# tuneinsight/lattigo

Hardware: AMD Instinct MI355X
Metric: ciphertext-mul+relin ops/s (higher is better)
Workload: dtype u64; 1 GPU; BGV logN=15, 12 Q-limbs [55,45x11] + 3 P-limbs [55x3], T=65537: ct x ct MulRelin (tensor + gadget product + ModDown), inputs resident in HBM; batch_per_gpu=256, logN=15, L=12, alpha=3, beta=4, parallelism=1 independent replicas, ciphertext-sharded

## Files before the change

### lattigo_amd/csrc/api.cpp

```cpp
#include <hip/hip_runtime.h>

#include <algorithm>
#include <atomic>
#include <chrono>
#include <condition_variable>
#include <deque>
#include <functional>
#include <cstdarg>
#include <cstdio>
#include <cstring>
#include <map>
#include <memory>
#include <tuple>
#include <mutex>
#include <shared_mutex>
#include <string>
#include <thread>
#include <unordered_map>
#include <unordered_set>
#include <cstdlib>
#include <vector>
#include <dlfcn.h>
#include <pthread.h>
#include <sched.h>
// ... 3025 lines not shown
    return mx != 0 && modup_f64_raw_ok(be.Q->logN, nsrc, mx);
}
struct MacDigits {
    const uint64_t *dec = nullptr;
    size_t bs = 0, ds = 0;
    bool raw = false, own_reduce = true;
};
struct TensorIn {
    View a0, a1, b0, b1;
    const uint64_t *ts;
};
struct LazyArgs {
    View cx;
    int B = 0;
    View c0Q, c0P, c1Q, c1P;
    bool cx_canonical = false;
    const TensorIn *tin = nullptr;
    const KsScatter *giant = nullptr;
    MacDigits *pending = nullptr;
};
int ks_mac_f64(Evaluator &ev, int levelQ, const Evk &k, const KsRoute &r, const LazyArgs &m, const MacDigits &dec, const NttMacEpilogue *epi) {
    BasisExtender &be = *ev.be;
    const hipStream_t st = be.ctx->stream;
    const int levelP = k.nPk - 1, N = be.Q->N;
    NttMacArgs a{};
    a.beta = base_rns_size(levelQ, levelP);
    key_product_limbs(a, be, k, levelQ, levelP, 2);
    a.dec_dstride = dec.ds;
    a.key_kstride = (size_t)(k.nQk + k.nPk) * N;
    a.key_dstride = 2 * a.key_kstride;
    a.own_alpha = levelP + 1;
    a.own_nq = levelQ + 1;
    a.own_reduce = dec.own_reduce ? 1 : 0;
    a.dec_f64 = dec.raw ? 1 : 0;
    a.q_out_f64 = 0;
    const View decv{const_cast<uint64_t *>(dec.dec), dec.bs};
    if (epi) {
        NttMacEpilogue e = *epi;
        for (int i = 0; i < a.nlimbs; i++) { e.sp[i] = epi->sp[a.out_limb[i]]; e.tsp[i] = epi->tsp[a.out_limb[i]]; }
        HIP_TRY(launch_ntt_mac_f64(be.qp, a, decv, m.cx, k.keyd, m.c0Q, m.c0P, m.c1Q, m.c1P, m.B, st, &e));
        return HE_OK;
    }
    if (!r.acc_q_f64) {
        HIP_TRY(launch_ntt_mac_f64(be.qp, a, decv, m.cx, k.keyd, m.c0Q, m.c0P, m.c1Q, m.c1P, m.B, st, nullptr, m.giant));
        return HE_OK;
    }
    NttMacArgs aq = a, ap = a;
    key_product_limbs(aq, be, k, levelQ, -1, 2);
    key_product_limbs(ap, be, k, -1, levelP, 2);
    aq.q_out_f64 = 1;
    HIP_TRY(launch_ntt_mac_f64(be.qp, aq, decv, m.cx, k.keyd, m.c0Q, m.c0P, m.c1Q, m.c1P, m.B, st));
    HIP_TRY(launch_ntt_mac_f64(be.qp, ap, decv, m.cx, k.keyd, m.c0Q, m.c0P, m.c1Q, m.c1P, m.B, st));
    return HE_OK;
}
struct KsCall {
    KsRoute route;
    const FusedPlan *dec = nullptr, *md = nullptr;
};
int rgsw_nj(const Evk &k, int i) { return k.pw2 ? k.nj[i] : 1; }
int window_products_core(Evaluator &ev, int levelQ, const Evk &k, const LazyArgs &a, bool reduce_wide) {
    BasisExtender &be = *ev.be;
    const int levelP = k.nPk - 1, N = be.Q->N, B = a.B;
    int beta = 0;
    for (int i = 0; i <= levelQ; i++) beta += rgsw_nj(k, i);
    const size_t wq = (size_t)B * (levelQ + 1) * N, ds = (size_t)(be.LQ + be.LP) * N, bs = (size_t)beta * ds;
    View inv{be.ctx->arena_take(wq), (size_t)(levelQ + 1) * N};
// ... 24 lines not shown
    return ks_inner(ev, levelQ, levelP, View{dec, bs}, ds, k, a.c0Q, a.c0P, a.c1Q, a.c1P, B);
}
int gadget_product_lazy_core(Evaluator &ev, int levelQ, const Evk &k, const KsCall &c, const LazyArgs &a) {
    BasisExtender &be = *ev.be;
    const KsRoute &r = c.route;
    const int levelP = k.nPk - 1, N = be.Q->N, B = a.B;
    const int beta = key_beta(k, levelQ);
    const size_t wq = (size_t)B * (levelQ + 1) * N, ds = (size_t)(be.LQ + be.LP) * N, bs = (size_t)beta * ds;
    const View cx = a.cx;
    if (a.tin) {
        LimbTab tt;
        QPLimb l[kMaxLimbs];
        uint64_t tsv[kMaxLimbs];
        tt.n = qp_limbs(be, levelQ, -1, r.prod_prologue ? 1 : 0, l);
        for (int i = 0; i < tt.n; i++) {
            tt.in_limb[i] = tt.out_limb[i] = tt.mod[i] = l[i].mod;
            tsv[i] = a.tin->ts[l[i].mod];
        }
        if (tt.n > 0)
            HIP_TRY(launch_tensor(be.qp, tt, tsv, a.tin->a0, a.tin->a1, a.tin->b0, a.tin->b1, View{nullptr, 0}, View{nullptr, 0}, cx, B, be.ctx->stream));
    }
    if (r.digits == KS_DIGITS_WINDOWS) return window_products_core(ev, levelQ, k, a, false);
    uint64_t *cxinv = be.ctx->arena_take(wq);
    uint64_t *dec = be.ctx->arena_take((size_t)B * bs);
    View inv{cxinv, (size_t)(levelQ + 1) * N};
    if (r.digits == KS_DIGITS_UNFUSED) {
        HIP_TRY(be_ntt(be, ident_tab(levelQ + 1), cx, inv, B, true, NTT_REDUCE_INPUT));
        TRY(decompose_ntt_into(ev, levelQ, levelP, levelP + 1, cx, inv, View{dec, bs}, ds, B));
        return ks_inner(ev, levelQ, levelP, View{dec, bs}, ds, k, a.c0Q, a.c0P, a.c1Q, a.c1P, B);
    }
    if (r.prod_prologue) {
        NttProdIn pin;
        pin.a = a.tin->a1; pin.b = a.tin->b1; pin.c = cx;
        for (int i = 0; i <= levelQ; i++) pin.ts[i] = a.tin->ts[i];
        HIP_TRY(launch_ntt_rows(be.qp, ident_tab(levelQ + 1), cx, inv, B, true, 0, be.ctx->stream, nullptr, &pin));
    } else {
        HIP_TRY(launch_ntt_rows(be.qp, ident_tab(levelQ + 1), cx, inv, B, true, a.cx_canonical ? 0 : NTT_REDUCE_INPUT, be.ctx->stream));
    }
    if (!r.mac_f64) {
        TRY(decompose_fused(ev, *c.dec, levelQ, levelP, levelP + 1, inv, View{dec, bs}, B));
        return ks_inner(ev, levelQ, levelP, View{dec, bs}, ds, k, a.c0Q, a.c0P, a.c1Q, a.c1P, B, &cx, levelP + 1, 0, 0, -1, a.giant);
    }
    int max_nsrc = 1;
    for (const FusedGroup &g : c.dec->groups) max_nsrc = std::max(max_nsrc, g.nsrc);
    const MacDigits digits{dec, bs, ds, f64_raw_ok(be, levelQ, levelP, max_nsrc), !a.cx_canonical};
    TRY(decompose_fused(ev, *c.dec, levelQ, levelP, levelP + 1, inv, View{dec, bs}, B, 1, digits.raw));
    TRY(ks_inner(ev, levelQ, levelP, View{dec, bs}, ds, k, a.c0Q, a.c0P, a.c1Q, a.c1P, B, &cx, levelP + 1, 1, 0, -1, a.giant));
    if (r.moddown == KS_MD_FUSED_MAC) {
        *a.pending = digits;
        return HE_OK;
    }
    return ks_mac_f64(ev, levelQ, k, r, a, digits, nullptr);
}
int moddown_front_fused(Evaluator &ev, const FusedPlan &plan, int levelQ, int levelP, View accP, View sP, View sQ, int nb, bool canonical, bool *raw) {
    BasisExtender &be = *ev.be;
    hipStream_t st = be.ctx->stream;
    HIP_TRY(launch_ntt_rows(be.qp, ident_tab(levelP + 1, 0, 0, be.LQ), accP, sP, nb, true, canonical ? 0 : NTT_REDUCE_INPUT, st));
    const FusedGroup &g = plan.groups[0];
    *raw = f64_raw_ok(be, levelQ, -1, g.nsrc);
    HIP_TRY(launch_modup_fused(be.qp, g.dev, 1, g.nsrc, g.dst_classes, sP, sQ, sQ, nb, st, *raw, g.total_limbs));
    return HE_OK;
}
void moddown_epilogue(NttEpilogue &epi, const BasisExtender &be, int levelP, const LimbTab &tab, View y) {
    for (int i = 0; i < tab.n; i++) epi.s[i] = be.Q->moduli[tab.mod[i]] - be.md_ptoq[levelP][tab.mod[i]];
    epi.y = y; epi.has_w = false; epi.w = y;
}
// ... 69 lines not shown
    epi.has_w = g.add0 != nullptr; epi.w = g.add0 ? *g.add0 : a0Q;
    epi.y_small_f64 = r.acc_q_f64;
    epi.zsplit = B; epi.out2 = g.out1; epi.y2 = a1Q; epi.has_w2 = g.add1 != nullptr; epi.w2 = g.add1 ? *g.add1 : a1Q;
    if (g.tin) {
        epi.tensor = true; epi.has_w = epi.has_w2 = false;
        epi.ta0 = g.tin->a0; epi.ta1 = g.tin->a1; epi.tb0 = g.tin->b0; epi.tb1 = g.tin->b1;
        for (int i = 0; i < ti.n; i++) epi.ts[i] = g.tin->ts[ti.mod[i]];
    }
    if (mac_epilogue) {
        NttMacEpilogue me;
        me.scatter_ginv = g.scatter_ginv;
        me.ext = sQ; me.ext_f64 = raw;
        me.out0 = g.out0; me.out1 = g.out1;
        me.has_w0 = g.add0 != nullptr && !g.tin; me.has_w1 = g.add1 != nullptr && !g.tin;
        me.w0 = g.add0 ? *g.add0 : g.out0; me.w1 = g.add1 ? *g.add1 : g.out1;
        me.tensor = g.tin != nullptr;
        if (g.tin) { me.ta0 = g.tin->a0; me.ta1 = g.tin->a1; me.tb0 = g.tin->b0; me.tb1 = g.tin->b1; }
        for (int i = 0; i <= levelQ; i++) {
            const ModConst &m = be.Q->sub[i].mc;
            me.sp[i] = (double)imform(be.Q->moduli[i] - be.md_ptoq[levelP][i], m.q, m.qinv);
            me.tsp[i] = g.tin ? (double)imform(imform(g.tin->ts[i], m.q, m.qinv), m.q, m.qinv) : 0.0;
        }
        TRY(ks_mac_f64(ev, levelQ, k, r, lazy, pending, &me));
    }
    if (ti.n > 0) HIP_TRY(launch_ntt_rows(be.qp, ti, sQ, g.out0, 2 * B, false, (raw && !mac_epilogue) ? NTT_INPUT_F64 : 0, st, &epi));
    return HE_OK;
}
int ks_call(Evaluator &ev, KsForm form, int levelQ, const Evk &k, KsAlias alias, KsCall *out) {
    static const bool no_mac_epilogue = env_flag("HERING_NO_MAC_EPILOGUE");
    static const bool no_prod_prologue = env_flag("HERING_NO_PROD_PROLOGUE");
    static const bool no_tensor_epilogue = env_flag("HERING_NO_TENSOR_EPILOGUE");
    static const bool no_auto_scatter = env_flag("HERING_NO_AUTO_SCATTER");
    static const bool no_giant_fusion = env_flag("HERING_NO_GIANT_FUSION");
    const BasisExtender &be = *ev.be;
    const int logN = be.Q->logN;
    KsFacts f;
    f.form = form; f.ring_type = be.type; f.levelP = k.nPk - 1;
    f.pw2 = k.pw2 != 0; f.keyd = k.keyd != nullptr; f.f64_tables = be.d_twdi != nullptr;
    for (int j = 0; j < k.nPk; j++) f.p_class2 = f.p_class2 || be.small[be.LQ + j] == 2;
    const bool lazy = form == KS_LAZY || form == KS_GIANT_STEP || form == KS_AUTOMORPHISM_HOISTED_LAZY;
    if (k.nPk > 0 && !k.pw2 && form != KS_HOISTED && form != KS_AUTOMORPHISM_HOISTED_LAZY) TRY(get_dec_plan(ev, levelQ, k.nPk - 1, k.nPk, &out->dec));
    if (k.nPk > 0 && !lazy) TRY(get_md_plan(ev, levelQ, k.nPk - 1, &out->md));
    f.dec_ok = out->dec && out->dec->ok; f.md_ok = out->md && out->md->ok;
    f.prod_in_supported = ntt_prod_in_supported(logN); f.scatter_supported = epilogue_scatter_supported(logN);
    f.mac_epilogue_supported = ntt_mac_epilogue_supported(logN); f.mac_giant_supported = ntt_mac_giant_supported(logN);
    f.alias = alias;
    f.no_mac_epilogue = no_mac_epilogue; f.no_prod_prologue = no_prod_prologue; f.no_tensor_epilogue = no_tensor_epilogue;
    f.no_auto_scatter = no_auto_scatter; f.no_giant_fusion = no_giant_fusion;
    out->route = ks_route(f);
    return HE_OK;
}
int key_switch(Evaluator &ev, KsForm form, int levelQ, const Evk &k, KsAlias alias, const GpArgs &g) {
    KsCall c;
    TRY(ks_call(ev, form, levelQ, k, alias, &c));
    return gadget_product_core(ev, levelQ, k, c, g);
}
void ks_request(CoReq &q, int op, std::shared_ptr<Evaluator> ev, std::shared_ptr<Evk> k, int level, KsForm form, KsAlias alias) {
    q.op = op; q.obj = ev.get(); q.key = k.get(); q.par[0] = level;
    q.keep.push_back(ev); q.keep.push_back(k);
    if (!k || form == KS_FORM_COUNT) return;
    q.tables_ok = [ev, k, form, level, alias](bool *ok) -> int {
        KsCall c;
        TRY(ks_call(*ev, form, level, *k, alias, &c));
        *ok = c.route.tables_ok;
        return HE_OK;
    };
}
int check_key(const Evaluator &ev, const Evk &k, int &levelQ, const char *who) {
    if (k.ev.get() != &ev) return fail(HE_EINVAL, "%s: key belongs to another evaluator", who);
    if (levelQ < 0) return fail(HE_EINVAL, "%s: negative level", who);
    levelQ = std::min(levelQ, k.nQk - 1);
    return HE_OK;
}
int check_decomp(const Evaluator &ev, const Decomp &dec, int levelQ, int levelP, const char *who) {
    if (dec.ev.get() != &ev) return fail(HE_EINVAL, "%s: decomposition buffer belongs to another evaluator", who);
    if (dec.fillQ < 0) return fail(HE_EINVAL, "%s: decomposition buffer was never filled", who);
    if (levelP != dec.fillP || levelQ > dec.fillQ || base_rns_size(levelQ, levelP) > dec.fill_beta)
        return fail(HE_EINVAL, "%s: decomposition buffer holds %d digits of level (%d,%d), (%d,%d) requested", who, dec.fill_beta,
                    dec.fillQ, dec.fillP, levelQ, levelP);
    return HE_OK;
}
// ... 2146 lines not shown
```

### lattigo_amd/csrc/kernels.h

```cpp
#pragma once

#include <hip/hip_runtime.h>
#include <stdint.h>
#include <cstdlib>

#include "modarith.h"

namespace he {

inline bool env_flag(const char *name) {
    const char *v = std::getenv(name);
    return v != nullptr && std::atoi(v) != 0;
}
constexpr int kMaxLimbs = 64;
constexpr int kMaxLogN = 20;

struct LimbTab {
    int n;
    uint8_t in_limb[kMaxLimbs];
    uint8_t out_limb[kMaxLimbs];
    uint8_t mod[kMaxLimbs];
};

struct View {
// ... 13 lines not shown
    const double *twd_fwd;
    const double *twd_inv;
    const uint64_t *tws_fwd = nullptr;
};

enum NttFlags {
    NTT_REDUCE_INPUT = 1,
    NTT_LAZY_OUT = 2,
    NTT_ADD_SCALAR = 4,
    NTT_INPUT_F64 = 8,
};
struct NttEpilogue;
hipError_t launch_ntt(const RingDev &r, const LimbTab &tab, View in, View out, int batch, bool inverse, int flags,
                      hipStream_t s, const uint64_t *io_scalar = nullptr, const NttEpilogue *epi = nullptr);
struct NttEpilogue {
    View y, w;
    bool has_w;
    uint64_t s[kMaxLimbs];
    bool y_small_f64 = false;
    bool y_reduce = false;
    int zsplit = 0;
    View out2, y2, w2;
    bool has_w2 = false;
    bool tensor = false;
    View ta0, ta1, tb0, tb1;
    uint64_t ts[kMaxLimbs];
    bool has_dst = false;
    View dst;
    uint32_t scatter_ginv = 0;
};
struct NttProdIn {
    View a, b, c;
    uint64_t ts[kMaxLimbs];
};
int ntt_row_bits(int logN);
bool ntt_prod_in_supported(int logN);
bool epilogue_scatter_supported(int logN);
hipError_t launch_ntt_rows(const RingDev &r, const LimbTab &tab, View in, View out, int batch, bool inverse, int flags,
                           hipStream_t s, const NttEpilogue *epi = nullptr, const NttProdIn *prod = nullptr);

hipError_t launch_ci_fold(const RingDev &r, const LimbTab &tab, View in, View out, int batch, bool inverse, bool reduce_input,
                          hipStream_t s);

hipError_t launch_ci_intt_lazy_ref(const RingDev &r, const ModConst &mc_host, int mod, View in, View out, int batch, hipStream_t s);

enum EwOp {
    EW_ADD = 0, EW_ADD_LAZY, EW_SUB, EW_SUB_LAZY,
    EW_MUL_BARRETT, EW_MUL_BARRETT_LAZY, EW_MUL_BARRETT_THEN_ADD, EW_MUL_BARRETT_THEN_ADD_LAZY,
    EW_MUL_MONT, EW_MUL_MONT_LAZY, EW_MUL_MONT_LAZY_THEN_NEG,
    EW_MUL_MONT_THEN_ADD, EW_MUL_MONT_THEN_ADD_LAZY, EW_MUL_MONT_LAZY_THEN_ADD_LAZY,
    EW_MUL_MONT_THEN_SUB, EW_MUL_MONT_THEN_SUB_LAZY, EW_MUL_MONT_LAZY_THEN_SUB_LAZY,
    EW_NEG = 100, EW_REDUCE, EW_REDUCE_LAZY, EW_MFORM, EW_MFORM_LAZY, EW_IMFORM, EW_COPY,
    EW_ZERO,
    EW_ADD_SCALAR = 200,
    EW_SUB_SCALAR,
    EW_MUL_SCALAR_MONT,
    EW_MUL_SCALAR_MONT_THEN_ADD,
    EW_ADD_SCALAR_LAZY,
    EW_SUB_THEN_MUL_SCALAR_MONT_2Q = 300,
    EW_DIVROUND_COEFF,
    EW_SUBMUL2Q_THEN_ADD,
};
struct ScalarTab {
    uint64_t s[kMaxLimbs];
    uint64_t s2[kMaxLimbs];
};
// ... 100 lines not shown
    int own_nq;
};
struct KsScatter {
    uint32_t ginv = 0;
    View add0{nullptr, 0};
    uint64_t add_s[kMaxLimbs];
    int plain = 0;
    View add0P{nullptr, 0};
    int accumulate = 0;
};
hipError_t launch_ks_inner(const RingDev &r, const KsArgs &a, View dec, View own, const uint64_t *key, View out0Q,
                           View out0P, View out1Q, View out1P, int batch, hipStream_t s, const KsScatter *sc = nullptr);

constexpr int kMaxDiag = 64;
struct DiagMacArgs {
    int n, nlimbs, accumulate;
    int mod0;
    const uint64_t *pt[kMaxDiag], *c0[kMaxDiag], *c1[kMaxDiag];
    const uint32_t *index[kMaxDiag];
    size_t pt_bs[kMaxDiag], c0_bs[kMaxDiag], c1_bs[kMaxDiag];
    const size_t *term_tab = nullptr;
    int term_rows = 3;
};
hipError_t launch_diag_mac(const RingDev &r, const DiagMacArgs &a, View out0, View out1, int batch, hipStream_t s);

struct NttMacArgs {
    int beta, nlimbs;
    uint8_t dec_limb[kMaxLimbs], key_limb[kMaxLimbs], out_limb[kMaxLimbs], out_view[kMaxLimbs], mod[kMaxLimbs];
    size_t dec_dstride, key_kstride, key_dstride;
    int own_alpha, own_nq;
    int dec_f64;
    int own_reduce;
    int q_out_f64;
};
struct NttMacEpilogue {
    View ext;
    bool ext_f64 = false;
    View out0, out1;
    bool has_w0 = false, has_w1 = false;
    View w0, w1;
    bool tensor = false;
    View ta0, ta1, tb0, tb1;
    double sp[kMaxLimbs], tsp[kMaxLimbs];
    uint32_t scatter_ginv = 0;
};
bool ntt_mac_epilogue_supported(int logN);
struct KsScatter;
hipError_t launch_ntt_mac_f64(const RingDev &r, const NttMacArgs &a, View dec, View own, const double *keyd, View out0Q,
                              View out0P, View out1Q, View out1P, int batch, hipStream_t s, const NttMacEpilogue *epi = nullptr,
                              const KsScatter *giant = nullptr);
bool ntt_mac_giant_supported(int logN);
hipError_t launch_key_to_f64(const RingDev &r, const uint64_t *key, double *keyd, int nblocks, const uint8_t *limb_mod_host,
                             int nlimbs, hipStream_t s);

struct RingSwitchIO {
    View in, out;
    View in2{nullptr, 0}, out2{nullptr, 0};
    int zsplit = -1;
};
hipError_t launch_ring_degree_fold_ntt(const RingDev &large, const LimbTab &tab, const uint64_t *gapinv_mont, RingSwitchIO io,
                                       int n_small, int log_gap, int batch, hipStream_t s);
hipError_t launch_ring_degree_replicate_ntt(const LimbTab &tab, RingSwitchIO io, int n_small, int log_gap, int batch, hipStream_t s);
hipError_t launch_ring_degree_stride(const LimbTab &tab, RingSwitchIO io, int n_small, int log_gap, bool up, int batch, hipStream_t s);
hipError_t launch_ci_bridge_fold(const RingDev &moduli, const LimbTab &tab, RingSwitchIO io, int n, int batch, hipStream_t s);
hipError_t launch_ci_bridge_unfold(const LimbTab &tab, RingSwitchIO io, int n, int batch, hipStream_t s);

// ... 32 lines not shown
```

### lattigo_amd/csrc/kernels.hip

```cpp
#include "kernels.h"

#include <atomic>
#include <cstdio>
#include <cstdlib>
#include <type_traits>
#include <mutex>
#include <unordered_map>
#include <vector>

namespace he {

namespace {
struct ProfRec { int id; hipEvent_t e0, e1; double bytes; };
struct ProfState { std::vector<ProfRec> recs; };
std::mutex g_prof_mu;
std::atomic<int> g_prof_active{0};
std::unordered_map<hipStream_t, ProfState> g_prof;
std::vector<hipEvent_t> g_prof_pool;
hipEvent_t prof_event_locked() {
    if (!g_prof_pool.empty()) { hipEvent_t e = g_prof_pool.back(); g_prof_pool.pop_back(); return e; }
    hipEvent_t e;
    (void)hipEventCreate(&e);
    return e;
}
// ... 172 lines not shown

struct NttArgs {
    const uint64_t *in;
    uint64_t *out;
    size_t in_bs, out_bs;
    const ModConst *mc;
    const uint64_t *tw;
    const double *twd;
    int N;
    int a;
    int flags;
    int scale;
    LimbTab tab;
    int epi;
    const uint64_t *epi_y, *epi_w;
    size_t epi_y_bs, epi_w_bs;
    uint64_t epi_s[kMaxLimbs];
    int zsplit;
    int epi2;
    uint64_t *out2;
    size_t out2_bs;
    const uint64_t *epi_y2, *epi_w2;
    size_t epi_y2_bs, epi_w2_bs;
    int epi_tensor;
    const uint64_t *ta0, *ta1, *tb0, *tb1;
    size_t ta0_bs, ta1_bs, tb0_bs, tb1_bs;
    uint64_t epi_ts[kMaxLimbs];
    uint64_t io_s[kMaxLimbs];
    int epi_y_f64;
    int epi_y_reduce;
    int nbatch, iters;
    int nbatch_prof = 0;
    int tprod = 0;
    unsigned sc_ginv = 0;
    int sc_logN = 0;
    const size_t *in_tab = nullptr;
    int cb = 0;
    const size_t *out_tab = nullptr, *out2_tab = nullptr, *epi_w_tab = nullptr, *epi_w2_tab = nullptr;
    const size_t *ta0_tab = nullptr, *ta1_tab = nullptr, *tb0_tab = nullptr, *tb1_tab = nullptr;
    const size_t *epi_y_tab = nullptr, *epi_y2_tab = nullptr;
};

__device__ __forceinline__ int lds_phys(int e) { return e + (e >> 4); }

__device__ __forceinline__ void wave_lds_sync() {
    __builtin_amdgcn_fence(__ATOMIC_RELEASE, "wavefront");
    __builtin_amdgcn_wave_barrier();
    __builtin_amdgcn_fence(__ATOMIC_ACQUIRE, "wavefront");
}
__device__ __forceinline__ void rows_sync(int sh) {
    if (sh <= 6) wave_lds_sync();
    else __syncthreads();
}
template <int T>
__device__ __forceinline__ int nat_e(int k, int tau) {
    constexpr int CH = T >= 64 ? 64 : T;
    return (tau / CH) * (16 * CH) + k * CH + (tau % CH);
}

int ntt_row_bits(int n) {
    return n <= 12 ? n : (n <= 15 ? 12 : 13);
}

template <int G4, bool INV, bool NC>
__device__ __forceinline__ void rows_round(uint64_t (&x)[16], const uint64_t *__restrict__ tw, int rowtw, int s0, int hi0,
                                           int tau, int sh, uint64_t q, uint64_t twoq, uint64_t qinv, const ModConst &mc,
                                           bool scale_last) {
    constexpr int g = G4, G = 1 << g, W = 16 / G;
    if constexpr (!INV) {
#pragma unroll
        for (int u = 0; u < g; u++) {
            const int d = 1 << (g - 1 - u);
#pragma unroll
            for (int w = 0; w < W; w++) {
                const int hi = (W == 1) ? hi0 : ((tau * W + w) >> sh);
                const int base = (rowtw << (s0 + u)) + (hi << u);
// ... 538 lines not shown
#pragma unroll
                for (int k = 0; k < 16; k++) wv[k] = ldnt(&wp[nat_e<T>(k, tau)]);
#pragma unroll
                for (int k = 0; k < 16; k++) {
                    const int e = nat_e<T>(k, tau);
                    const uint64_t v = canon_f64(modmul_f64(lds[lds_phys(e)] - yv[k], sp, q, qi), q, qi);
                    uint64_t *dp = &op[e];
                    if constexpr (SCAT) dp = op - (size_t)row * N2 + auto_dest((unsigned)(row * N2 + e), A.sc_ginv, A.sc_logN);
                    stnt(dp, cred(wv[k] + v, mc.q));
                }
            } else {
#pragma unroll
                for (int k = 0; k < 16; k++) {
                    const int e = nat_e<T>(k, tau);
                    uint64_t *dp = &op[e];
                    if constexpr (SCAT) dp = op - (size_t)row * N2 + auto_dest((unsigned)(row * N2 + e), A.sc_ginv, A.sc_logN);
                    stnt(dp, canon_f64(modmul_f64(lds[lds_phys(e)] - yv[k], sp, q, qi), q, qi));
                }
            }
        } else {
#pragma unroll
            for (int k = 0; k < 16; k++) {
                const int e = nat_e<T>(k, tau);
                dst[e] = canon_f64(lds[lds_phys(e)], q, qi);
            }
        }
    } else {
        if constexpr (TP) {
            const size_t off = (size_t)il * A.N + (size_t)row * N2;
            const uint64_t *pa = A.ta1 + voff(A.ta1_tab, A.ta1_bs, bzi) + off, *pb = A.tb1 + voff(A.tb1_tab, A.tb1_bs, bzi) + off;
            uint64_t *pc = A.out2 + (size_t)bzi * A.out2_bs + off;
            const double tsp = (double)imform(imform(A.epi_ts[y], mc.q, mc.qinv), mc.q, mc.qinv);
            const uint64_t twoq_u = mc.q << 1;
#pragma unroll
            for (int h = 0; h < 2; h++) {
                uint64_t ua[8], ub[8];
#pragma unroll
                for (int k = 0; k < 8; k++) { const int e = nat_e<T>(8 * h + k, tau); ua[k] = ldnt(&pa[e]); ub[k] = ldnt(&pb[e]); }
                bool big = false;
#pragma unroll
                for (int k = 0; k < 8; k++) big = big || ua[k] >= twoq_u || ub[k] >= twoq_u;
                if (__any(big)) {
#pragma unroll
                    for (int k = 0; k < 8; k++) { ua[k] = bred_add_lazy(ua[k], mc.q, mc.brc0); ub[k] = bred_add_lazy(ub[k], mc.q, mc.brc0); }
                }
#pragma unroll
                for (int k = 0; k < 8; k++) {
                    const int e = nat_e<T>(8 * h + k, tau);
                    const double c = canon_f64d(modmul_f64(modmul_f64(u52_to_f64(ua[k]), u52_to_f64(ub[k]), q, qi), tsp, q, qi), q, qi);
                    stnt(&pc[e], f64_to_u52(c));
                    lds[lds_phys(e)] = c;
                }
            }
        } else {
        if (A.flags & NTT_REDUCE_INPUT) {
            const uint64_t twoq_u = mc.q << 1;
            bool big = false;
#pragma unroll
            for (int k = 0; k < 16; k++) big = big || nx[k] >= twoq_u;
            if (__any(big)) {
#pragma unroll
                for (int k = 0; k < 16; k++) nx[k] = bred_add_lazy(nx[k], mc.q, mc.brc0);
            }
        }
#pragma unroll
        for (int k = 0; k < 16; k++) lds[lds_phys(nat_e<T>(k, tau))] = u52_to_f64(nx[k]);
        }
        if constexpr (PIPE) if (bzi + 1 < b1) {
            const uint64_t *srcn = A.in + voff(A.in_tab, A.in_bs, bzi + 1) + in_off;
#pragma unroll
            for (int k = 0; k < 16; k++) nx[k] = ldnt(&srcn[nat_e<T>(k, tau)]);
        }
        rows_sync(0);
        if constexpr (GREM > 0) {
            constexpr int s0 = 4 * NR4;
            rows_lds_xfer_f64<LOGB, GREM>(x, lds, tau, s0, 0, false);
            rows_round_f64<GREM, true>(x, tw, rowtw, s0, 0, tau, 0, q, qi);
            rows_lds_xfer_f64<LOGB, GREM>(x, lds, tau, s0, 0, true);
            rows_sync(GREM);
        }
        double t16[15];
        if constexpr (NR4 > 0) rows_tw16_f64(t16, tw, rowtw, 4 * (NR4 - 1), tau >> (LOGB - 4 * NR4));
#pragma unroll 1
        for (int rho = NR4 - 1; rho >= 0; rho--) {
// ... 265 lines not shown
        return A.m.own_alpha > 0 && !it.isP && it.ql >= d * A.m.own_alpha && it.ql < (d + 1) * A.m.own_alpha;
    };
    const int nd = A.m.beta + (EPI ? 2 : 0);
    auto digit_src = [&](const Item &it, int d) -> const uint64_t * {
        if (EPI && d >= A.m.beta)
            return AA.e.ext + ((size_t)(d - A.m.beta) * AA.nbatch + it.bz) * AA.e.ext_bs + (size_t)it.ql * A.N + it.rowoff;
        return own_digit(it, d) ? A.own + voff(A.own_tab, A.own_bs, it.bz) + (size_t)it.ql * A.N + it.rowoff
                                : A.dec + it.bz * A.dec_bs + (size_t)d * A.m.dec_dstride + (size_t)it.ql * A.N + it.rowoff;
    };
    const unsigned pw_addr = lds_byte_addr(pbuf) + wv * 8192u;
    auto dma_digit = [&](const uint64_t *src, unsigned lane) {
        const uint64_t *gp = src + ((lane >> 5) * T + 64u * wv + 2u * (lane & 31u));
#pragma unroll
        for (int j = 0; j < 8; j++) glds16(gp + (size_t)j * 2 * T, pw_addr + (unsigned)j * 1024u);
    };

    unsigned t = 0;
    unsigned w = item_of(0);
    if (w == ~0u) return;
    Item cur = decode(w);
    dma_digit(digit_src(cur, 0), lane);
    for (;;) {
        const unsigned t_cur = t; (void)t_cur;
        MAC_STAMP2(0);
        double acc0[16], acc1[16];
#pragma unroll
        for (int k = 0; k < 16; k++) { acc0[k] = 0.0; acc1[k] = 0.0; }
        const double q = cur.q, qi = cur.qi;
        if (tau < 240u) {
            const unsigned hi = tau / 15u, idx = tau - hi * 15u, u = 31u - (unsigned)__builtin_clz(idx + 1u), j = idx + 1u - (1u << u);
            tw1s[tau] = cur.tw[((unsigned)cur.rowtw << (4 + u)) + (hi << u) + j];
        }
        bool more = false;
        auto round0 = [&](double (&x)[16]) {
            double t0[15];
#pragma unroll
            for (int u = 0; u < 4; u++)
#pragma unroll
                for (int j = 0; j < (1 << u); j++) t0[(1 << u) - 1 + j] = ldcd(cur.tw, (size_t)(((unsigned)cur.rowtw << u) + j));
            rows_round16_f64<false>(x, t0, q, qi);
        };
        auto round1 = [&](double (&x)[16], unsigned tau) {
            rows_lds_xfer_f64<LOGB, 4>(x, lds, tau, 4, LOGB - 8, false);
            {
                double t1[15];
                const double *tp = tw1s + (tau >> (LOGB - 8)) * 15u;
#pragma unroll
                for (int i = 0; i < 15; i++) t1[i] = tp[i];
                rows_round16_f64<false>(x, t1, q, qi);
            }
            rows_lds_xfer_f64<LOGB, 4>(x, lds, tau, 4, LOGB - 8, true);
            rows_sync(LOGB - 8);
            rows_lds_xfer_f64<LOGB, 4>(x, lds, tau, 8, LOGB - 12, false);
        };
        auto transform = [&](int nk, double (&x)[16], unsigned tau, unsigned lane, const uint64_t *nsrc, const double *k0p,
                             const double *k1p, double (&kk0)[16], double (&kk1)[16]) {
            double t2[15];
            rows_tw16_f64(t2, cur.tw, cur.rowtw, 8, tau >> (LOGB - 12));
            __builtin_amdgcn_sched_barrier(0);
            asm volatile("s_waitcnt lgkmcnt(0)" ::: "memory");
            if (nsrc) dma_digit(nsrc, lane);
            __builtin_amdgcn_sched_barrier(0);
            round0(x);
            __syncthreads();
            rows_lds_xfer_f64<LOGB, 4>(x, lds, tau, 0, LOGB - 4, true);
            __syncthreads();
// ... 23 lines not shown
            w = item_of(++t);
            more = w != ~0u;
            return more ? digit_src(decode(w), 0) : nullptr;
        };
        for (int d = 0; d < A.m.beta; d++) {
            const bool is_own = own_digit(cur, d);
            unsigned tau_d = threadIdx.x;
            asm volatile("" : "+v"(tau_d));
            const unsigned tau = tau_d, lane = tau & 63u;
            const double *pw = pbuf + wv * 1024u + lane;
            MAC_STAMP2(1 + d * 12 + 0);
            asm volatile("s_waitcnt vmcnt(0)" ::: "memory");
            uint64_t xi[16];
#pragma unroll
            for (int k = 0; k < 16; k++) xi[k] = (uint64_t)__double_as_longlong(pw[k * 64]);
            double x[16];
            if (is_own && A.m.own_reduce) {
#pragma unroll
                for (int k = 0; k < 16; k++) xi[k] = bred_add_lazy(xi[k], ldc(reinterpret_cast<const uint64_t *>(A.mc + cur.mi), 0), ldc(reinterpret_cast<const uint64_t *>(A.mc + cur.mi), 2));
            }
            if (A.m.dec_f64 && !is_own) {
#pragma unroll
                for (int k = 0; k < 16; k++) x[k] = __longlong_as_double((long long)xi[k]);
            } else {
#pragma unroll
                for (int k = 0; k < 16; k++) x[k] = u52_to_f64(xi[k]);
            }
            MAC_STAMP2(1 + d * 12 + 1);
            const uint64_t *nsrc = next_src(d);
            const double *k0p = cur.kbase + (size_t)d * A.m.key_dstride + tau, *k1p = k0p + A.m.key_kstride;
            double kk0[16], kk1[16];
            if (!is_own) {
                transform(2, x, tau, lane, nsrc, k0p, k1p, kk0, kk1);
            } else {
                asm volatile("s_waitcnt lgkmcnt(0)" ::: "memory");
                if (nsrc) dma_digit(nsrc, lane);
                __builtin_amdgcn_sched_barrier(0);
#pragma unroll
                for (int k = 0; k < 16; k++) kk0[k] = k0p[(unsigned)(k * T)];
#pragma unroll
                for (int k = 0; k < 16; k++) kk1[k] = k1p[(unsigned)(k * T)];
                __builtin_amdgcn_sched_barrier(0);
                __syncthreads();
                rows_lds_xfer_f64<LOGB, 4>(x, lds, tau, 0, LOGB - 4, true);
                __syncthreads();
                mac_final_xfer<LOGB>(x, lds, tau, false);
            }
            MAC_STAMP2(1 + d * 12 + 8);
#pragma unroll
            for (int k = 0; k < 16; k++) acc0[k] += modmul_f64(x[k], kk0[k], q, qi);
            MAC_STAMP2(1 + d * 12 + 9);
#pragma unroll
            for (int k = 0; k < 16; k++) acc1[k] += modmul_f64(x[k], kk1[k], q, qi);
            MAC_STAMP2(1 + d * 12 + 10);
        }
        if constexpr (EPI && TEN && LOGB == 12) {
            unsigned tau_d = threadIdx.x;
            asm volatile("" : "+v"(tau_d));
            const unsigned tau = tau_d, lane = tau & 63u;
            const double *pw = pbuf + wv * 1024u + lane;
            MAC_STAMP2(48);
            asm volatile("s_waitcnt vmcnt(0)" ::: "memory");
            double xA[16], xB[16];
            uint64_t wB[16];
#pragma unroll
            for (int k = 0; k < 16; k++) xA[k] = pw[k * 64];
            const uint64_t *srcB = digit_src(cur, A.m.beta + 1) + tau;
            const uint64_t *nsrc = next_src(A.m.beta + 1);
#pragma unroll
            for (int k = 0; k < 16; k++) wB[k] = ldnt(&srcB[(unsigned)(k * T)]);
            double t2[15];
            rows_tw16_f64(t2, cur.tw, cur.rowtw, 8, tau);
            __builtin_amdgcn_sched_barrier(0);
            asm volatile("s_waitcnt lgkmcnt(0)" ::: "memory");
            if (nsrc) dma_digit(nsrc, lane);
            __builtin_amdgcn_sched_barrier(0);
            if (!AA.e.ext_f64) {
#pragma unroll
                for (int k = 0; k < 16; k++) xA[k] = u52_to_f64((uint64_t)__double_as_longlong(xA[k]));
// ... 221 lines not shown
                ext_pass(std::integral_constant<int, 1>{});
            } else {
#pragma unroll 1
                for (int c = 0; c < 2; c++) ext_pass(c);
            }
        }
        const int ol = cur.out_limb;
        uint64_t *o0 = nullptr, *o1 = nullptr;
        unsigned tau_t = threadIdx.x;
        asm volatile("" : "+v"(tau_t));
        const unsigned tau = tau_t;
        if constexpr (!EPI) {
            o0 = (cur.isP ? A.o0P + voff(A.oP0_tab, A.oP0_bs, cur.bz) : A.o0Q + voff(A.oQ0_tab, A.oQ0_bs, cur.bz)) + (size_t)ol * A.N + cur.rowoff + tau;
            o1 = (cur.isP ? A.o1P + voff(A.oP1_tab, A.oP1_bs, cur.bz) : A.o1Q + voff(A.oQ1_tab, A.oQ1_bs, cur.bz)) + (size_t)ol * A.N + cur.rowoff + tau;
        }
        [[maybe_unused]] uint64_t gs_av[16], gs_p0[16], gs_p1[16];
        [[maybe_unused]] const uint64_t *gs_ap = nullptr;
        if constexpr (!EPI && SCAT) {
            __builtin_amdgcn_sched_barrier(0);
            const size_t src = cur.rowoff + tau;
            if (AA.e.has_w0) gs_ap = (cur.isP ? AA.e.w1 + meoff(AA.e, ME_W1, AA.e.w1_bs, cur.bz, AA.nbatch) : AA.e.w0 + meoff(AA.e, ME_W0, AA.e.w0_bs, cur.bz, AA.nbatch)) + (size_t)ol * A.N + src;
            if (gs_ap) {
#pragma unroll
                for (int k = 0; k < 16; k++) gs_av[k] = ldnt(&gs_ap[(unsigned)(k * T)]);
            }
            if (AA.e.gs_accum) {
                const uint64_t *b0p = o0 - src;
#pragma unroll
                for (int k = 0; k < 16; k++) gs_p0[k] = b0p[auto_dest((unsigned)src + (unsigned)(k * T), AA.e.sc_ginv, AA.e.sc_logN)];
            }
            __builtin_amdgcn_sched_barrier(0);
        }
        if constexpr (!EPI) {
            auto to_natural = [&](double (&a)[16]) {
                mac_final_xfer<LOGB>(a, lds, tau, true);
                __syncthreads();
#pragma unroll
                for (int k = 0; k < 16; k++) a[k] = lds[lds_phys(k * T + tau)];
            };
            to_natural(acc0);
            if constexpr (SCAT) {
                const uint64_t qu = ldc(reinterpret_cast<const uint64_t *>(A.mc + cur.mi), 0);
                const size_t src = cur.rowoff + tau;
                uint64_t *b0p = o0 - src;
                const uint64_t *b1p = o1 - src;
                const bool accum = AA.e.gs_accum != 0;
                if (accum) {
#pragma unroll
                    for (int k = 0; k < 16; k++) gs_p1[k] = b1p[auto_dest((unsigned)src + (unsigned)(k * T), AA.e.sc_ginv, AA.e.sc_logN)];
                }
                __builtin_amdgcn_sched_barrier(0);
#pragma unroll
                for (int k = 0; k < 16; k++) {
                    uint64_t v0 = canon_f64(acc0[k], q, qi);
                    if (gs_ap) v0 = cred(v0 + gs_av[k], qu);
                    if (accum) v0 += gs_p0[k];
                    stnt(&b0p[auto_dest((unsigned)src + (unsigned)(k * T), AA.e.sc_ginv, AA.e.sc_logN)], v0);
                }
            }
            __syncthreads();
            to_natural(acc1);
        }
        if constexpr (EPI) {
            (void)o0; (void)o1; (void)ol;
        } else if constexpr (SCAT) {
            const size_t src = cur.rowoff + tau;
// ... 30 lines not shown
        int dev = 0, n = 0;
        if (hipGetDevice(&dev) != hipSuccess || hipDeviceGetAttribute(&n, hipDeviceAttributeMultiprocessorCount, dev) != hipSuccess || n <= 0)
            n = 256;
        return (unsigned)n;
    }();
    return logb >= 13 ? cus : 2u * cus;
}

bool ntt_prod_in_supported(int logN) {
    const int b = ntt_row_bits(logN);
    return b == 12 || b == 13;
}
bool epilogue_scatter_supported(int logN) {
    const int b = ntt_row_bits(logN);
    return b == 12 || b == 13;
}
bool ntt_mac_epilogue_supported(int logN) {
    const int b = ntt_row_bits(logN);
    return b == 12 || b == 13;
}
bool ntt_mac_giant_supported(int logN) {
    const int b = ntt_row_bits(logN);
    return b == 12 || b == 13;
}
hipError_t launch_ntt_mac_f64(const RingDev &r, const NttMacArgs &a, View dec, View own, const double *keyd, View out0Q,
                              View out0P, View out1Q, View out1P, int batch, hipStream_t s, const NttMacEpilogue *epi,
                              const KsScatter *giant) {
    if (a.nlimbs <= 0 || batch <= 0) return hipSuccess;
    if (!r.twd_fwd || !keyd) return hipErrorInvalidValue;
    if (giant && (epi || a.q_out_f64 || !giant->ginv || !ntt_mac_giant_supported(r.logN))) return hipErrorInvalidValue;
    if (dec.tab || (epi && epi->ext.tab) || (a.q_out_f64 && !no_tab({out0Q, out1Q}))) return hipErrorInvalidValue;
    const int b = ntt_row_bits(r.logN), aa = r.logN - b;
    if (epi && !ntt_mac_epilogue_supported(r.logN)) return hipErrorInvalidValue;
    NttMacKArgs A{};
    A.dec = dec.p; A.dec_bs = dec.bstride; A.own = own.p; A.own_bs = own.bstride; A.own_tab = own.tab; A.keyd = keyd;
    A.o0Q = out0Q.p; A.o0P = out0P.p; A.o1Q = out1Q.p; A.o1P = out1P.p;
    A.oQ0_bs = out0Q.bstride; A.oP0_bs = out0P.bstride; A.oQ1_bs = out1Q.bstride; A.oP1_bs = out1P.bstride;
    A.oQ0_tab = out0Q.tab; A.oP0_tab = out0P.tab; A.oQ1_tab = out1Q.tab; A.oP1_tab = out1P.tab;
    A.mc = r.mc; A.twd = r.twd_fwd; A.N = r.N; A.a = aa; A.m = a;
    double mac_bytes = ((double)a.beta * batch + 2.0 * a.beta + 2.0 * batch) * a.nlimbs * (double)r.N * 8.0;
    if (epi) mac_bytes += (2.0 + (epi->tensor ? 4.0 : (epi->has_w0 ? 1.0 : 0.0) + (epi->has_w1 ? 1.0 : 0.0))) * batch * a.nlimbs * (double)r.N * 8.0;
    if (epi || giant || b >= 12) {
        NttMacDmaArgs D;
        D.k = A;
        D.e = MacEpiK{};
        if (epi) {
            D.e.ext = epi->ext.p; D.e.ext_bs = epi->ext.bstride; D.e.ext_f64 = epi->ext_f64 ? 1 : 0;
            D.e.out0 = epi->out0.p; D.e.out0_bs = epi->out0.bstride; D.e.out1 = epi->out1.p; D.e.out1_bs = epi->out1.bstride;
            D.e.has_w0 = epi->has_w0 ? 1 : 0; D.e.has_w1 = epi->has_w1 ? 1 : 0;
            D.e.w0 = epi->w0.p; D.e.w0_bs = epi->w0.bstride; D.e.w1 = epi->w1.p; D.e.w1_bs = epi->w1.bstride;
            D.e.tensor = epi->tensor ? 1 : 0;
            if (epi->scatter_ginv && epi->tensor) return hipErrorInvalidValue;
            D.e.sc_ginv = epi->scatter_ginv; D.e.sc_logN = r.logN;
            D.e.ta0 = epi->ta0.p; D.e.ta0_bs = epi->ta0.bstride; D.e.ta1 = epi->ta1.p; D.e.ta1_bs = epi->ta1.bstride;
            D.e.tb0 = epi->tb0.p; D.e.tb0_bs = epi->tb0.bstride; D.e.tb1 = epi->tb1.p; D.e.tb1_bs = epi->tb1.bstride;
            {
                const View *vs[8] = {&epi->out0, &epi->out1, &epi->w0, &epi->w1, &epi->ta0, &epi->ta1, &epi->tb0, &epi->tb1};
                const size_t *base = nullptr;
                for (const View *v : vs) if (v->tab && (!base || v->tab < base)) base = v->tab;
                D.e.etab = base;
                D.e.etab_rows = 0xFFFFFFFFu;
                for (int i = 0; i < 8 && base; i++) {
                    if (!vs[i]->tab) continue;
                    const size_t d = (size_t)(vs[i]->tab - base);
                    if (d % (size_t)batch != 0 || d / (size_t)batch >= 15) return hipErrorInvalidValue;
                    D.e.etab_rows = (D.e.etab_rows & ~(0xFu << (4 * i))) | ((unsigned)(d / (size_t)batch) << (4 * i));
// ... 56 lines not shown
    dim3 grid(batch, a.nlimbs, 1u << aa);
    ProfScope ps(K_NTT_MAC_F64, s, mac_bytes);
#define HE_MAC_CASE(B)                                                                                      \
    case B:                                                                                                 \
        if (a.q_out_f64) hipLaunchKernelGGL((ntt_mac_f64_kernel<B, true>), grid, dim3((1 << B) / 16), 0, s, A);  \
        else hipLaunchKernelGGL((ntt_mac_f64_kernel<B, false>), grid, dim3((1 << B) / 16), 0, s, A);             \
        break;
    switch (b) {
        HE_MAC_CASE(4) HE_MAC_CASE(5) HE_MAC_CASE(6) HE_MAC_CASE(7) HE_MAC_CASE(8) HE_MAC_CASE(9) HE_MAC_CASE(10)
        HE_MAC_CASE(11)
        default: return hipErrorInvalidValue;
    }
#undef HE_MAC_CASE
    return hipGetLastError();
}

struct KeyF64Args {
    const uint64_t *key;
    double *keyd;
    const ModConst *mc;
    int N, nlimbs;
    int rowbits;
    uint8_t mod[kMaxLimbs];
};
__global__ void __launch_bounds__(256) key_to_f64_kernel(KeyF64Args A) {
    const int x = blockIdx.x * blockDim.x + threadIdx.x;
    if (x >= A.N) return;
    const int l = blockIdx.y;
    const size_t base = ((size_t)blockIdx.z * A.nlimbs + l) * A.N;
    const ModConst m = A.mc[A.mod[l]];
    size_t dst = (size_t)x;
    if (A.rowbits > 0) {
        const unsigned e = (unsigned)x & ((1u << A.rowbits) - 1u), T = 1u << (A.rowbits - 4);
        dst = (size_t)((unsigned)x - e) + (e & 15u) * T + (e >> 4);
    }
    A.keyd[base + dst] = (m.q >> kF64Bits) == 0 ? (double)imform(A.key[base + x], m.q, m.qinv) : 0.0;
}
hipError_t launch_key_to_f64(const RingDev &r, const uint64_t *key, double *keyd, int nblocks, const uint8_t *limb_mod_host,
                             int nlimbs, hipStream_t s) {
    KeyF64Args A{};
    A.key = key; A.keyd = keyd; A.mc = r.mc; A.N = r.N; A.nlimbs = nlimbs;
    A.rowbits = ntt_row_bits(r.logN) >= 12 ? ntt_row_bits(r.logN) : 0;
    for (int i = 0; i < nlimbs; i++) A.mod[i] = limb_mod_host[i];
    dim3 grid((unsigned)((r.N + 255) / 256), nlimbs, nblocks), block(256);
    hipLaunchKernelGGL(key_to_f64_kernel, grid, block, 0, s, A);
    return hipGetLastError();
}

template <int LOGA, bool INV, bool INNER = false>
__global__ void __launch_bounds__(256) ntt_cols_kernel(NttArgs A) {
    constexpr int R = 1 << LOGA;
    const int cbits = INNER ? A.cb : 0;
    const int N2 = (A.N >> cbits) >> LOGA;
    const int cg = blockIdx.x * blockDim.x + threadIdx.x;
    if (cg >= (A.N >> LOGA)) return;
    const int blk = INNER ? cg >> __builtin_ctz((unsigned)N2) : 0, c = INNER ? cg & (N2 - 1) : cg;
    const int rowtw = INNER ? (1 << cbits) + blk : 1;
    const int y = blockIdx.y;
    const int il = A.tab.in_limb[y], ol = A.tab.out_limb[y], mi = A.tab.mod[y];
    const ModConst mc = A.mc[mi];
    const uint64_t q = mc.q, qinv = mc.qinv, twoq = mc.q << 1;
    const uint64_t *__restrict__ tw = A.tw + (size_t)mi * A.N;
    const size_t e0 = (size_t)blk * ((size_t)N2 << LOGA) + c;
    const uint64_t *__restrict__ src = A.in + voff(A.in_tab, A.in_bs, blockIdx.z) + (size_t)il * A.N + e0;
    uint64_t *__restrict__ dst = A.out + voff(A.out_tab, A.out_bs, blockIdx.z) + (size_t)ol * A.N + e0;

    uint64_t x[R];
// ... 267 lines not shown
        B.scale = 1;
        return launch_cols<true>(a_out, gcols, B, s);
    }
    return hipSuccess;
}

hipError_t launch_ntt_rows(const RingDev &r, const LimbTab &tab, View in, View out, int batch, bool inverse, int flags,
                           hipStream_t s, const NttEpilogue *epi, const NttProdIn *prod) {
    if (tab.n <= 0 || batch <= 0) return hipSuccess;
    const int n = r.logN;
    if (n < 4 || n > 17) return hipErrorInvalidValue;
    if (epi && inverse) return hipErrorInvalidValue;
    if (prod && (!inverse || !r.twd_inv || !ntt_prod_in_supported(n))) return hipErrorInvalidValue;
    if ((in.tab && epi && epi->tensor) || (prod && prod->c.tab)) return hipErrorInvalidValue;
    const int b = ntt_row_bits(n), a = n - b;
    NttArgs A{};
    A.mc = r.mc; A.N = r.N; A.a = a; A.tab = tab;
    A.epi = 0; A.epi_y = A.epi_w = nullptr; A.epi_y_bs = A.epi_w_bs = 0;
    A.zsplit = 0; A.epi2 = 0; A.out2 = nullptr; A.out2_bs = 0; A.epi_y2 = A.epi_w2 = nullptr; A.epi_y2_bs = A.epi_w2_bs = 0;
    A.epi_y_f64 = 0; A.epi_y_reduce = 0;
    for (int i = 0; i < tab.n; i++) A.io_s[i] = 0;
    A.epi_tensor = 0;
    if (epi) {
        if (epi->tensor && (epi->zsplit <= 0 || batch != 2 * epi->zsplit)) return hipErrorInvalidValue;
        set_epilogue(A, *epi, tab.n);
    }
    A.in = in.p; A.in_bs = in.bstride; A.in_tab = in.tab; A.out = out.p; A.out_bs = out.bstride; A.out_tab = out.tab;
    A.flags = flags;
    if (prod) {
        A.tprod = 1;
        A.ta1 = prod->a.p; A.ta1_bs = prod->a.bstride; A.tb1 = prod->b.p; A.tb1_bs = prod->b.bstride;
        A.ta1_tab = prod->a.tab; A.tb1_tab = prod->b.tab;
        A.out2 = prod->c.p; A.out2_bs = prod->c.bstride;
        for (int i = 0; i < tab.n; i++) A.epi_ts[i] = prod->ts[i];
    }
    dim3 grows(A.epi_tensor ? (unsigned)((epi->zsplit + 7) / 8 * 16) : (unsigned)batch, tab.n, 1u << a);
    if (!inverse) {
        A.tw = r.tw_fwd; A.twd = r.twd_fwd; A.scale = 0;
        return launch_rows<false>(b, grows, A, r.host_small, s);
    }
    A.tw = r.tw_inv; A.twd = r.twd_inv; A.scale = (a == 0);
    return launch_rows<true>(b, grows, A, r.host_small, s);
}

struct CiFoldArgs {
    const uint64_t *in;
    uint64_t *out;
    size_t in_bs, out_bs;
    const ModConst *mc;
    int N, inverse, reduce_input;
    uint8_t in_limb[kMaxLimbs], out_limb[kMaxLimbs], mod[kMaxLimbs];
};
__global__ void __launch_bounds__(256) ci_fold_kernel(CiFoldArgs A) {
    const int j = blockIdx.x * blockDim.x + threadIdx.x;
    if (j > A.N / 2) return;
    const ModConst m = A.mc[A.mod[blockIdx.y]];
    const uint64_t q = m.q, qinv = m.qinv, twoq = m.q << 1;
    const uint64_t *in = A.in + (size_t)blockIdx.z * A.in_bs + (size_t)A.in_limb[blockIdx.y] * A.N;
    uint64_t *out = A.out + (size_t)blockIdx.z * A.out_bs + (size_t)A.out_limb[blockIdx.y] * A.N;
    const int jy = (A.N - j) & (A.N - 1);
    uint64_t a = in[j], b = in[jy];
    if (A.reduce_input) { a = bred_add_lazy(a, q, m.brc0); b = bred_add_lazy(b, q, m.brc0); }
    if (!A.inverse) {
        const uint64_t F = m.pad0;
        if (j == 0) { out[0] = a; return; }
        const uint64_t oa = a + twoq - mred_lazy(b, F, q, qinv), ob = b + twoq - mred_lazy(a, F, q, qinv);
// ... 2061 lines not shown
```

### lattigo_amd/csrc/ks_route.h

```cpp
#pragma once

enum KsForm { KS_GADGET_PRODUCT, KS_LAZY, KS_HOISTED, KS_AUTOMORPHISM, KS_AUTOMORPHISM_HOISTED, KS_AUTOMORPHISM_HOISTED_LAZY, KS_GIANT_STEP,
              KS_MUL_RELIN, KS_FORM_COUNT };
struct KsAlias {
    bool out_is_operand = false, out_is_addend = false, crossed = false;
};
struct KsFacts {
    KsForm form = KS_GADGET_PRODUCT;
    int ring_type = 0, levelP = -1;
    bool pw2 = false, keyd = false, p_class2 = false, f64_tables = false;
    bool dec_ok = false, md_ok = false;
    bool prod_in_supported = false, scatter_supported = false, mac_epilogue_supported = false, mac_giant_supported = false;
    KsAlias alias;
    bool no_mac_epilogue = false, no_prod_prologue = false, no_tensor_epilogue = false, no_auto_scatter = false, no_giant_fusion = false;
};
enum KsDigits { KS_DIGITS_WINDOWS, KS_DIGITS_FUSED, KS_DIGITS_UNFUSED, KS_DIGITS_GIVEN };
enum KsModDown { KS_MD_NONE, KS_MD_UNFUSED, KS_MD_FUSED_ROWS, KS_MD_FUSED_MAC };
enum KsAuto { KS_AUTO_NONE, KS_AUTO_EPILOGUE_SCATTER, KS_AUTO_KS_SCATTER, KS_AUTO_GATHERS };
struct KsRoute {
    KsDigits digits = KS_DIGITS_UNFUSED;
    KsModDown moddown = KS_MD_NONE;
    KsAuto automorphism = KS_AUTO_NONE;
    bool mac_f64 = false, prod_prologue = false, acc_q_f64 = false, tensor_epilogue = false, giant_fused = false, tables_ok = false;
};
inline KsRoute ks_route(const KsFacts &f) {
    KsRoute r;
    const bool hasP = f.levelP >= 0, standard = f.ring_type == 0;
    const bool given = f.form == KS_HOISTED || f.form == KS_AUTOMORPHISM_HOISTED || f.form == KS_AUTOMORPHISM_HOISTED_LAZY;
    const bool lazy = f.form == KS_LAZY || f.form == KS_AUTOMORPHISM_HOISTED_LAZY || f.form == KS_GIANT_STEP;
    const bool automorphism = f.form == KS_AUTOMORPHISM || f.form == KS_AUTOMORPHISM_HOISTED;

    r.digits = given ? KS_DIGITS_GIVEN : f.pw2 ? KS_DIGITS_WINDOWS : f.dec_ok ? KS_DIGITS_FUSED : KS_DIGITS_UNFUSED;
    r.mac_f64 = r.digits == KS_DIGITS_FUSED && f.keyd;

    const bool auto_alias = f.alias.out_is_operand || f.alias.out_is_addend || f.alias.crossed;
    if (automorphism)
        r.automorphism = (!f.no_auto_scatter && !auto_alias && f.md_ok && f.scatter_supported) ? KS_AUTO_EPILOGUE_SCATTER : KS_AUTO_GATHERS;
    if (f.form == KS_AUTOMORPHISM_HOISTED_LAZY) r.automorphism = (!f.no_auto_scatter && standard && !auto_alias) ? KS_AUTO_KS_SCATTER : KS_AUTO_GATHERS;
    r.giant_fused = f.form == KS_GIANT_STEP && !f.no_auto_scatter && !f.no_giant_fusion && r.digits == KS_DIGITS_FUSED &&
                    (!f.keyd || f.mac_giant_supported);
    if (f.form == KS_GIANT_STEP) r.automorphism = r.giant_fused ? KS_AUTO_KS_SCATTER : KS_AUTO_GATHERS;

    if (!lazy && hasP) {
        r.moddown = f.md_ok ? KS_MD_FUSED_ROWS : KS_MD_UNFUSED;
        const bool writes_operand = f.alias.out_is_operand && r.automorphism != KS_AUTO_GATHERS;
        if (f.md_ok && r.mac_f64 && !f.no_mac_epilogue && f.mac_epilogue_supported && !f.p_class2 && !writes_operand) r.moddown = KS_MD_FUSED_MAC;
    }
    r.acc_q_f64 = r.moddown == KS_MD_FUSED_ROWS && r.mac_f64;
    r.tensor_epilogue = f.form == KS_MUL_RELIN && f.md_ok && !f.alias.out_is_addend && !f.no_tensor_epilogue;
    r.prod_prologue = r.tensor_epilogue && r.digits == KS_DIGITS_FUSED && f.f64_tables && f.prod_in_supported && !f.no_prod_prologue;

    switch (f.form) {
    case KS_LAZY: case KS_GIANT_STEP: r.tables_ok = r.digits == KS_DIGITS_FUSED; break;
    case KS_HOISTED: r.tables_ok = standard; break;
    case KS_GADGET_PRODUCT: r.tables_ok = f.dec_ok && f.md_ok && !f.alias.out_is_operand && !f.alias.crossed; break;
    case KS_AUTOMORPHISM: case KS_AUTOMORPHISM_HOISTED: r.tables_ok = f.dec_ok && f.md_ok && !auto_alias; break;
    case KS_MUL_RELIN: r.tables_ok = f.md_ok; break;
    default: break;
    }
    return r;
}
```

Baseline: 43560 ctxt-mul+relin ops/s.

## Store tensor-product c1 in MAC accumulator order to skip own-digit LDS transposes

When the product prologue and f64 MAC are both active with 4096-element rows, the NTT product prologue writes the c1 term in the MAC kernel's accumulator (transposed) order through an extra LDS shuffle. The MAC kernel can then load the own digit directly, skipping two syncthreads and two LDS transfer passes per tile. This adds a wave-level LDS exchange in the prologue, plus a conditional barrier to keep LDS reuse safe, and is gated by an environment flag and a row-size check.

```diff
diff --git a/lattigo_amd/csrc/api.cpp b/lattigo_amd/csrc/api.cpp
--- a/lattigo_amd/csrc/api.cpp
+++ b/lattigo_amd/csrc/api.cpp
@@ -3081,6 +3081,7 @@
     a.own_alpha = levelP + 1;
     a.own_nq = levelQ + 1;
     a.own_reduce = dec.own_reduce ? 1 : 0;
+    a.own_order = r.own_acc_order ? 1 : 0;
     a.dec_f64 = dec.raw ? 1 : 0;
     a.q_out_f64 = 0;
     const View decv{const_cast<uint64_t *>(dec.dec), dec.bs};
@@ -3171,6 +3172,7 @@
     if (r.prod_prologue) {
         NttProdIn pin;
         pin.a = a.tin->a1; pin.b = a.tin->b1; pin.c = cx;
+        pin.acc_order = r.own_acc_order;
         for (int i = 0; i <= levelQ; i++) pin.ts[i] = a.tin->ts[i];
         HIP_TRY(launch_ntt_rows(be.qp, ident_tab(levelQ + 1), cx, inv, B, true, 0, be.ctx->stream, nullptr, &pin));
     } else {
@@ -3306,6 +3308,7 @@
     static const bool no_tensor_epilogue = env_flag("HERING_NO_TENSOR_EPILOGUE");
     static const bool no_auto_scatter = env_flag("HERING_NO_AUTO_SCATTER");
     static const bool no_giant_fusion = env_flag("HERING_NO_GIANT_FUSION");
+    static const bool no_own_order = env_flag("HERING_NO_OWN_ORDER");
     const BasisExtender &be = *ev.be;
     const int logN = be.Q->logN;
     KsFacts f;
@@ -3320,7 +3323,8 @@
     f.mac_epilogue_supported = ntt_mac_epilogue_supported(logN); f.mac_giant_supported = ntt_mac_giant_supported(logN);
     f.alias = alias;
     f.no_mac_epilogue = no_mac_epilogue; f.no_prod_prologue = no_prod_prologue; f.no_tensor_epilogue = no_tensor_epilogue;
-    f.no_auto_scatter = no_auto_scatter; f.no_giant_fusion = no_giant_fusion;
+    f.no_auto_scatter = no_auto_scatter; f.no_giant_fusion = no_giant_fusion; f.no_own_order = no_own_order;
+    f.rows_4096 = ntt_row_bits(logN) == 12;
     out->route = ks_route(f);
     return HE_OK;
 }
diff --git a/lattigo_amd/csrc/kernels.h b/lattigo_amd/csrc/kernels.h
--- a/lattigo_amd/csrc/kernels.h
+++ b/lattigo_amd/csrc/kernels.h
@@ -69,6 +69,7 @@
 struct NttProdIn {
     View a, b, c;
     uint64_t ts[kMaxLimbs];
+    bool acc_order = false;
 };
 int ntt_row_bits(int logN);
 bool ntt_prod_in_supported(int logN);
@@ -235,6 +236,7 @@
     int dec_f64;
     int own_reduce;
     int q_out_f64;
+    int own_order;
 };
 struct NttMacEpilogue {
     View ext;
diff --git a/lattigo_amd/csrc/kernels.hip b/lattigo_amd/csrc/kernels.hip
--- a/lattigo_amd/csrc/kernels.hip
+++ b/lattigo_amd/csrc/kernels.hip
@@ -228,6 +228,7 @@
     int nbatch, iters;
     int nbatch_prof = 0;
     int tprod = 0;
+    int tprod_acc_order = 0;
     unsigned sc_ginv = 0;
     int sc_logN = 0;
     const size_t *in_tab = nullptr;
@@ -238,6 +239,7 @@
 };
 
 __device__ __forceinline__ int lds_phys(int e) { return e + (e >> 4); }
+__device__ __forceinline__ unsigned acc_order_pos(unsigned e, unsigned T) { return (e & 15u) * T + (e >> 4); }
 
 __device__ __forceinline__ void wave_lds_sync() {
     __builtin_amdgcn_fence(__ATOMIC_RELEASE, "wavefront");
@@ -842,6 +844,7 @@
             uint64_t *pc = A.out2 + (size_t)bzi * A.out2_bs + off;
             const double tsp = (double)imform(imform(A.epi_ts[y], mc.q, mc.qinv), mc.q, mc.qinv);
             const uint64_t twoq_u = mc.q << 1;
+            const bool acc_order = GREM == 0 && A.tprod_acc_order;
 #pragma unroll
             for (int h = 0; h < 2; h++) {
                 uint64_t ua[8], ub[8];
@@ -858,8 +861,17 @@
                 for (int k = 0; k < 8; k++) {
                     const int e = nat_e<T>(8 * h + k, tau);
                     const double c = canon_f64d(modmul_f64(modmul_f64(u52_to_f64(ua[k]), u52_to_f64(ub[k]), q, qi), tsp, q, qi), q, qi);
-                    stnt(&pc[e], f64_to_u52(c));
+                    if (!acc_order) stnt(&pc[e], f64_to_u52(c));
                     lds[lds_phys(e)] = c;
+                }
+                if (acc_order) {
+                    wave_lds_sync();
+                    const unsigned t0 = ((unsigned)tau & ~63u) + 32u * (unsigned)h + ((unsigned)tau & 31u), k0 = ((unsigned)tau >> 5) & 1u;
+                    double cc[8];
+#pragma unroll
+                    for (int j = 0; j < 8; j++) cc[j] = lds[lds_phys((int)(16u * t0 + 2u * (unsigned)j + k0))];
+#pragma unroll
+                    for (int j = 0; j < 8; j++) stnt(&pc[acc_order_pos(16u * t0 + 2u * (unsigned)j + k0, T)], f64_to_u52(cc[j]));
                 }
             }
         } else {
@@ -1191,6 +1203,7 @@
             tw1s[tau] = cur.tw[((unsigned)cur.rowtw << (4 + u)) + (hi << u) + j];
         }
         bool more = false;
+        [[maybe_unused]] bool tile_open = false;
         auto round0 = [&](double (&x)[16]) {
             double t0[15];
 #pragma unroll
@@ -1280,6 +1293,7 @@
             double kk0[16], kk1[16];
             if (!is_own) {
                 transform(2, x, tau, lane, nsrc, k0p, k1p, kk0, kk1);
+                tile_open = true;
             } else {
                 asm volatile("s_waitcnt lgkmcnt(0)" ::: "memory");
                 if (nsrc) dma_digit(nsrc, lane);
@@ -1289,10 +1303,13 @@
 #pragma unroll
                 for (int k = 0; k < 16; k++) kk1[k] = k1p[(unsigned)(k * T)];
                 __builtin_amdgcn_sched_barrier(0);
-                __syncthreads();
-                rows_lds_xfer_f64<LOGB, 4>(x, lds, tau, 0, LOGB - 4, true);
-                __syncthreads();
-                mac_final_xfer<LOGB>(x, lds, tau, false);
+                if (LOGB != 12 || !A.m.own_order) {
+                    __syncthreads();
+                    rows_lds_xfer_f64<LOGB, 4>(x, lds, tau, 0, LOGB - 4, true);
+                    __syncthreads();
+                    mac_final_xfer<LOGB>(x, lds, tau, false);
+                    tile_open = true;
+                }
             }
             MAC_STAMP2(1 + d * 12 + 8);
 #pragma unroll
@@ -1580,6 +1597,7 @@
             __builtin_amdgcn_sched_barrier(0);
         }
         if constexpr (!EPI) {
+            if (LOGB == 12 && !tile_open) __syncthreads();
             auto to_natural = [&](double (&a)[16]) {
                 mac_final_xfer<LOGB>(a, lds, tau, true);
                 __syncthreads();
@@ -1676,6 +1694,7 @@
     if (dec.tab || (epi && epi->ext.tab) || (a.q_out_f64 && !no_tab({out0Q, out1Q}))) return hipErrorInvalidValue;
     const int b = ntt_row_bits(r.logN), aa = r.logN - b;
     if (epi && !ntt_mac_epilogue_supported(r.logN)) return hipErrorInvalidValue;
+    if (a.own_order && b != 12) return hipErrorInvalidValue;
     NttMacKArgs A{};
     A.dec = dec.p; A.dec_bs = dec.bstride; A.own = own.p; A.own_bs = own.bstride; A.own_tab = own.tab; A.keyd = keyd;
     A.o0Q = out0Q.p; A.o0P = out0P.p; A.o1Q = out1Q.p; A.o1P = out1P.p;
@@ -1798,7 +1817,7 @@
     size_t dst = (size_t)x;
     if (A.rowbits > 0) {
         const unsigned e = (unsigned)x & ((1u << A.rowbits) - 1u), T = 1u << (A.rowbits - 4);
-        dst = (size_t)((unsigned)x - e) + (e & 15u) * T + (e >> 4);
+        dst = (size_t)((unsigned)x - e) + acc_order_pos(e, T);
     }
     A.keyd[base + dst] = (m.q >> kF64Bits) == 0 ? (double)imform(A.key[base + x], m.q, m.qinv) : 0.0;
 }
@@ -2132,6 +2151,8 @@
         A.ta1 = prod->a.p; A.ta1_bs = prod->a.bstride; A.tb1 = prod->b.p; A.tb1_bs = prod->b.bstride;
         A.ta1_tab = prod->a.tab; A.tb1_tab = prod->b.tab;
         A.out2 = prod->c.p; A.out2_bs = prod->c.bstride;
+        if (prod->acc_order && b != 12) return hipErrorInvalidValue;
+        A.tprod_acc_order = prod->acc_order ? 1 : 0;
         for (int i = 0; i < tab.n; i++) A.epi_ts[i] = prod->ts[i];
     }
     dim3 grows(A.epi_tensor ? (unsigned)((epi->zsplit + 7) / 8 * 16) : (unsigned)batch, tab.n, 1u << a);
diff --git a/lattigo_amd/csrc/ks_route.h b/lattigo_amd/csrc/ks_route.h
--- a/lattigo_amd/csrc/ks_route.h
+++ b/lattigo_amd/csrc/ks_route.h
@@ -11,8 +11,10 @@
     bool pw2 = false, keyd = false, p_class2 = false, f64_tables = false;
     bool dec_ok = false, md_ok = false;
     bool prod_in_supported = false, scatter_supported = false, mac_epilogue_supported = false, mac_giant_supported = false;
+    bool rows_4096 = false;
     KsAlias alias;
     bool no_mac_epilogue = false, no_prod_prologue = false, no_tensor_epilogue = false, no_auto_scatter = false, no_giant_fusion = false;
+    bool no_own_order = false;
 };
 enum KsDigits { KS_DIGITS_WINDOWS, KS_DIGITS_FUSED, KS_DIGITS_UNFUSED, KS_DIGITS_GIVEN };
 enum KsModDown { KS_MD_NONE, KS_MD_UNFUSED, KS_MD_FUSED_ROWS, KS_MD_FUSED_MAC };
@@ -22,6 +24,7 @@
     KsModDown moddown = KS_MD_NONE;
     KsAuto automorphism = KS_AUTO_NONE;
     bool mac_f64 = false, prod_prologue = false, acc_q_f64 = false, tensor_epilogue = false, giant_fused = false, tables_ok = false;
+    bool own_acc_order = false;
 };
 inline KsRoute ks_route(const KsFacts &f) {
     KsRoute r;
@@ -50,6 +53,8 @@
     r.tensor_epilogue = f.form == KS_MUL_RELIN && f.md_ok && !f.alias.out_is_addend && !f.no_tensor_epilogue;
     r.prod_prologue = r.tensor_epilogue && r.digits == KS_DIGITS_FUSED && f.f64_tables && f.prod_in_supported && !f.no_prod_prologue;
 
+    r.own_acc_order = r.prod_prologue && r.mac_f64 && f.rows_4096 && !f.no_own_order;
+
     switch (f.form) {
     case KS_LAZY: case KS_GIANT_STEP: r.tables_ok = r.digits == KS_DIGITS_FUSED; break;
     case KS_HOISTED: r.tables_ok = standard; break;
```

Result: no change. 43720 ctxt-mul+relin ops/s (median of 6 runs) (+0.4%).
